# nicoRomeroCuruchet/DynamicProgramming

Hardware: AMD Instinct MI355X
Metric: state-action Bellman backups/sec (higher is better)
Workload: dtype f32; 1 GPU; double_pendulum_swingup 4D grid bins=80/dim (40960000 states) x 11 actions, gamma=0.999; step = 10 eval sweeps + 1 improve sweep = 860160000 backups; terminal states are counted in `value` (0 of 40960000: value_nonterminal leaves them out); states=40960000, nonterminal_states=40960000, actions=11, parallelism=state-range shards x1

## Files before the change

dynamicprogramming_amd/_native.py:

```python
from __future__ import annotations

import ctypes
import enum
import os
from pathlib import Path

import numpy as np

_PKG = Path(__file__).resolve().parent
LIB_PATH = _PKG / "libpi_mi355.so"
KERNEL_CACHE = Path(os.environ.get("PI_MI355_KERNEL_CACHE", str(_PKG / "_kcache")))

_f32p = ctypes.POINTER(ctypes.c_float)
_i32p = ctypes.POINTER(ctypes.c_int32)
_vp = ctypes.c_void_p

SIGNATURES = {
    "pi_abi_version": (ctypes.c_int, []),
    "pi_last_error": (ctypes.c_char_p, []),
    "pi_create": (_vp, [ctypes.c_int, ctypes.c_int, _i32p, _f32p, _f32p,
                        ctypes.POINTER(_f32p), _f32p, ctypes.c_int]),
    "pi_destroy": (None, [_vp]),
    "pi_compile": (ctypes.c_int, [_vp, ctypes.c_char_p, ctypes.c_char_p, ctypes.c_char_p,
                                  ctypes.c_size_t]),
    "pi_kernel_source": (ctypes.c_size_t, [_vp, ctypes.c_char_p, ctypes.c_char_p, ctypes.c_size_t]),
    "pi_eval_sweep": (ctypes.c_int, [_vp, _vp, _vp, _vp, _vp, ctypes.c_int64, ctypes.c_int64,
                                     ctypes.c_float, _vp, _vp]),
    "pi_eval_sweeps": (ctypes.c_int, [_vp, _vp, _vp, _vp, _vp, ctypes.c_int64, ctypes.c_int64,
                                      ctypes.c_float, ctypes.c_int, _vp, _vp]),
    "pi_policy_evaluation": (ctypes.c_int, [_vp, _vp, _vp, _vp, ctypes.c_float, ctypes.c_double, ctypes.c_int,
                                            ctypes.c_int, _vp, _vp, _vp, _vp]),
    "pi_policy_iteration": (ctypes.c_int, [_vp, _vp, _vp, _vp, ctypes.c_float, ctypes.c_double, ctypes.c_int,
                                           ctypes.c_int, ctypes.c_int, _vp, _vp, _vp]),
    "pi_improve_sweep": (ctypes.c_int, [_vp, _vp, _vp, _vp, ctypes.c_int64, ctypes.c_int64,
                                        ctypes.c_float, _vp, _vp]),
    "pi_value_sweep": (ctypes.c_int, [_vp, _vp, _vp, _vp, _vp, ctypes.c_int64, ctypes.c_int64,
                                      ctypes.c_float, _vp, _vp, _vp]),
    "pi_reach_planes": (ctypes.c_int, [_vp, _vp, ctypes.c_int64, ctypes.c_int64, ctypes.c_int, _vp, _vp]),
    "pi_reach_depth_max": (ctypes.c_int, [_vp]),
    "pi_reach_units": (ctypes.c_int, [_vp, _vp, ctypes.c_int64, ctypes.c_int64, ctypes.c_int, _vp, _vp]),
    "pi_comm_unique_id": (ctypes.c_int, [_vp]),
    "pi_comm_init": (ctypes.c_int, [_vp, ctypes.c_int, ctypes.c_int, _vp]),
    "pi_comm_init_local": (ctypes.c_int, [_vp, ctypes.c_int, ctypes.c_int, ctypes.c_char_p]),
    "pi_p2p_describe": (ctypes.c_int, [_vp, ctypes.c_int, ctypes.c_int, _vp, _vp, ctypes.c_int, _vp]),
    "pi_comm_init_p2p": (ctypes.c_int, [_vp, ctypes.c_int, ctypes.c_int, _vp, ctypes.c_char_p]),
    "pi_p2p_compile_check": (ctypes.c_int, [ctypes.c_char_p]),
    "pi_comm_destroy": (ctypes.c_int, [_vp]),
    "pi_comm_info": (ctypes.c_int, [_vp, ctypes.c_int]),
    "pi_allgather_V": (ctypes.c_int, [_vp, _vp, ctypes.c_int64, _vp]),
    "pi_allgather_policy": (ctypes.c_int, [_vp, _vp, ctypes.c_int64, _vp]),
# ... 16 lines not shown
    "pi_infer_destroy": (None, [_vp]),
    "pi_infer_set_policy": (ctypes.c_int, [_vp, _i32p, ctypes.c_int64, _f32p, ctypes.c_int]),
    "pi_infer_query": (ctypes.c_int, [_vp, _vp, ctypes.c_int64, _vp, _vp, _vp, _vp]),
    "pi_plan_schedule": (ctypes.c_int, [_vp, ctypes.c_int, ctypes.c_int64, ctypes.c_int64, ctypes.c_int64, ctypes.c_int,
                                        ctypes.POINTER(ctypes.c_uint64)]),
    "pi_set_option": (ctypes.c_int, [_vp, ctypes.c_int, ctypes.c_int64]),
    "pi_info": (ctypes.c_int64, [_vp, ctypes.c_int]),
    "pi_debug_report": (ctypes.c_int, [_vp, ctypes.POINTER(ctypes.c_uint32)]),
    "pi_prepare_mask": (ctypes.c_int, [_vp, _vp, _vp]),
    "pi_prepare_mask_range": (ctypes.c_int, [_vp, _vp, ctypes.c_int64, ctypes.c_int64, _vp]),
    "pi_live_list": (ctypes.c_int64, [_vp, _vp, ctypes.c_int64, _vp]),
    "pi_eval_begin": (ctypes.c_int, [_vp, _vp, _vp, _vp]),
    "pi_eval_end": (ctypes.c_int, [_vp]),
}

ABI_VERSION = 10
_lib = None
_load_error: Exception | None = None


class Info(enum.IntEnum):
    N_STATES = 0
    N_ACTIONS = 1
    DIMS = 2
    EVAL_CPW = 3
    EVAL_VGPRS = 4
    IMPROVE_VGPRS = 5
    COMPUTE_UNITS = 6
    CACHE_HIT = 7
    IMPROVE_CPW = 8
    CACHED_GRAPHS = 9
# ... 2 lines not shown
    IMPROVE_BLOCK = 12
    RESIDENT_STATES_PER_THREAD = 13
    RESIDENT_ENABLED = 14
    DEBUG_CHECKS = 15
    LIVE_STATES = 16
    EVAL_LIST_ENTRIES = 17
    MEMORY_ORDER = 18
    FLOW_WORKGROUPS = 19
    RECIPROCAL_DIV = 20
    XCD_ENABLED = 30
    XCD_EVALUATIONS = 31
    XCD_FALLBACKS = 32
    WHOLE_RUNS = 33
    WHOLE_RUN_AVAILABLE = 34
    STRIP_STATES = 35


class Option(enum.IntEnum):
    EVAL_CPW = 0
    IMPROVE_CPW = 1
    GRAPHS = 2
    RESIDENT = 3
    MEMORY_ORDER = 4
    BUILD_PUSH = 5
    KEEP_LIVE_LIST = 6
    STRIP_STATES = 7
    XCD_RUN_FAILED = 8


class XcdFailure(enum.IntEnum):
# ... 219 lines not shown
                          d_residual_log, stream=0):
        _check(lib().pi_policy_evaluation(self._h, V, policy, term, gamma, float(theta), int(max_sweeps),
                                          int(check_interval), d_sweeps, d_delta or None, d_residual_log,
                                          stream or None), "pi_policy_evaluation")

    def policy_iteration(self, V, policy, term, gamma, theta, max_eval_sweeps, check_interval, max_pi_iter, d_result,
                         d_iter_log, stream=0):
        _check(lib().pi_policy_iteration(self._h, V, policy, term, gamma, float(theta), int(max_eval_sweeps),
                                         int(check_interval), int(max_pi_iter), d_result, d_iter_log, stream or None),
               "pi_policy_iteration")

    def improve_sweep(self, V, policy, term, s_begin, s_end, gamma, d_changed=0, stream=0):
        _check(lib().pi_improve_sweep(self._h, V, policy, term, s_begin, s_end, gamma,
                                      d_changed or None, stream or None), "pi_improve_sweep")

    def value_sweep(self, V, Vnew, policy, term, s_begin, s_end, gamma, d_delta=0, d_changed=0, stream=0):
        _check(lib().pi_value_sweep(self._h, V, Vnew, policy, term, s_begin, s_end, gamma,
                                    d_delta or None, d_changed or None, stream or None), "pi_value_sweep")

    def reach_planes(self, term, s_begin, s_end, d_bitmap, stream=0, dim=0):
        _check(lib().pi_reach_planes(self._h, term, s_begin, s_end, int(dim), d_bitmap, stream or None),
               "pi_reach_planes")

    def reach_depth_max(self) -> int:
        return int(lib().pi_reach_depth_max(self._h))

    def reach_units(self, term, s_begin, s_end, depth, d_bitmap, stream=0):
        _check(lib().pi_reach_units(self._h, term, s_begin, s_end, int(depth), d_bitmap, stream or None),
               "pi_reach_units")

# ... 162 lines not shown
```

dynamicprogramming_amd/csrc/pi_api.cpp:

```cpp

#include "pi_internal.h"

#include <hip/hiprtc.h>

#include <algorithm>
#include <cmath>
#include <cstdio>
#include <cstdlib>
#include <cstring>
#include <fstream>
#include <map>
#include <mutex>
#include <sstream>
#include <sys/stat.h>
#include <unistd.h>

#ifndef PI_CSRC_DIR
#error "build with -DPI_CSRC_DIR=\"...\" and -DPI_INCLUDE_DIR=\"...\""
#endif
asm(".section .rodata\n"
    ".global pi_embedded_kernels\n"
    "pi_embedded_kernels:\n"
    ".incbin \"" PI_CSRC_DIR "/pi_sweep_kernels.hip\"\n"
    ".byte 0\n"
// ... 259 lines not shown
            }
        }
    }
    return Grid2{launch_blocks(block, count, cpw), 1u};
}

}

namespace {

using pi::Sched;
using pi::plan_launch;

unsigned int* delta_slots(pi_handle* h) { return h->d_slots; }
unsigned int* changed_slots(pi_handle* h) { return h->d_slots + kSlots; }

}

namespace pi {

int check_ready(const pi_handle* h) {
    if (!h) return fail("null handle");
    if (h->device < 0) return fail("host-only handle (device = -1) cannot launch kernels");
    if (!h->module) return fail("pi_compile has not been called on this handle");
    return 0;
}

int check_range(const pi_handle* h, int64_t s_begin, int64_t s_end) {
    if (s_begin < 0 || s_end < s_begin || s_end > h->n_states)
        return fail("state range [" + std::to_string(s_begin) + ", " + std::to_string(s_end) +
// ... 48 lines not shown
    for (int64_t w = a >> 6; w <= (b - 1) >> 6 && a < b; ++w) {
        uint64_t word = h->live_bits[(size_t)(w - word0)];
        while (word) {
            const int bit = __builtin_ctzll(word);
            word &= word - 1;
            const int64_t s = (w << 6) + bit;
            if (s >= a && s < b) out.push_back((int32_t)s);
        }
    }
}

int64_t live_list_total(const pi_handle* h, int64_t entries) {
    const int64_t range = h->live_hi - h->live_lo;
    if (range <= 0 || entries <= 0) return 0;
    return (int64_t)((double)entries * ((double)h->n_states / (double)range));
}

void drop_eval_list(pi_handle* h) {
    h->eval_count = -1;
    h->eval_policy = nullptr;
    h->eval_holds.clear();
}

int launch_eval_live(pi_handle* h, const float* V, float* Vnew, const int32_t* policy, int64_t first, int64_t count,
                     float gamma, bool want_delta, hipStream_t st, const int32_t* list, int64_t list_total) {
    if (count <= 0) return 0;
    const int32_t* live = (list ? list : h->d_live) + first;
    if (!list) list_total = live_list_total(h, h->live_count);
    long long cnt = count;
    const float* tab = h->d_tab;
// ... 125 lines not shown
    h->xcd = h->flow && xcd_wanted;
    h->xcd_ring = env_int("PI_MI355_XCD_RING", 64, 4, 1024);
    h->xcd_states = (int)(((n + 31) / 32 + 31) / 32 * 32);
    if (device >= 0) {
        pi::DeviceGuard guard(device);
        hipDeviceProp_t prop;
        hipError_t e = hipGetDeviceProperties(&prop, device);
        if (e == hipSuccess && std::string(prop.gcnArchName).rfind(kArch, 0) != 0) {
            fail(std::string("pi_create: device is ") + prop.gcnArchName +
                 ", this library is built for gfx950 only");
            return nullptr;
        }
        if (e == hipSuccess) e = hipMalloc((void**)&h->d_tab, h->tab.size() * sizeof(float));
        if (e == hipSuccess)
            e = hipMemcpy(h->d_tab, h->tab.data(), h->tab.size() * sizeof(float), hipMemcpyHostToDevice);
        if (e == hipSuccess) e = hipMalloc((void**)&h->d_slots, 2 * kSlots * sizeof(unsigned int));
        if (e == hipSuccess) e = hipMemset(h->d_slots, 0, 2 * kSlots * sizeof(unsigned int));
        if (e != hipSuccess) {
            fail(std::string("pi_create: ") + hipGetErrorString(e));
            if (h->d_tab) (void)hipFree(h->d_tab);
            if (h->d_slots) (void)hipFree(h->d_slots);
            return nullptr;
        }
        h->num_cu = prop.multiProcessorCount;
    } else {
        h->num_cu = 256;
    }
    return h.release();
}

void pi_destroy(pi_handle* h) {
    if (!h) return;
// ... 144 lines not shown
        (void)hipGetLastError();
        return fail("could not build the evaluation-sweep graph");
    }
    return 0;
}

}

extern "C" {

int pi_compile(pi_handle* h, const char* dynamics_src, const char* cache_dir, char* log,
               size_t log_len) {
    pi::fail("");
    if (log && log_len) log[0] = 0;
    if (!h || !dynamics_src) return fail("null argument");
    std::vector<char> image;
    if (pi::compile_image(build_source(h, dynamics_src), cache_dir, log, log_len, image, &h->cache_hit)) return 1;
    h->compiled = true;
    resolve_strip(h);
    h->dynamics_src = dynamics_src;
    h->has_cache_dir = cache_dir != nullptr;
    h->cache_dir = cache_dir ? cache_dir : "";
    return load_module(h, image);
}

int pi_eval_sweep(pi_handle* h, const float* V, float* Vnew, const int32_t* policy,
                  const uint8_t* term, int64_t s_begin, int64_t s_end, float gamma,
                  float* d_delta, void* stream) {
    if (check_ready(h) || check_range(h, s_begin, s_end)) return 1;
    if (!V || !Vnew || !policy) return fail("null device pointer");
    if (V == Vnew) return fail("V and Vnew must be different buffers (Jacobi sweep)");
    pi::DeviceGuard guard(h->device);
    hipStream_t st = (hipStream_t)stream;
    if (s_end == s_begin) {
        if (d_delta) PI_HIP(hipMemsetAsync(d_delta, 0, sizeof(float), st));
        return 0;
    }
    if (pi::launch_eval(h, V, Vnew, policy, term, s_begin, s_end, gamma, d_delta != nullptr, st)) return 1;
    return pi::finalize(h, d_delta, nullptr, st);
}

int pi_eval_sweeps(pi_handle* h, float* Va, float* Vb, const int32_t* policy,
                   const uint8_t* term, int64_t s_begin, int64_t s_end, float gamma,
                   int n_sweeps, float* d_delta, void* stream) {
    if (check_ready(h) || check_range(h, s_begin, s_end)) return 1;
    if (n_sweeps < 0) return fail("n_sweeps < 0");
    if (!Va || !Vb || !policy) return fail("null device pointer");
    if (Va == Vb) return fail("Va and Vb must be different buffers (Jacobi sweep)");
    if (n_sweeps == 0) return 0;
    pi::DeviceGuard guard(h->device);
    hipStream_t st = (hipStream_t)stream;
    if (s_end == s_begin) {
        if (d_delta) PI_HIP(hipMemsetAsync(d_delta, 0, sizeof(float), st));
        return 0;
    }
    if (h->f_resident && h->use_resident && n_sweeps >= 2 && s_begin == 0 && s_end == h->n_states) {
        const float* tab = h->d_tab;
        double theta = 0.0;
        int interval = 1;
        int* sweeps_out = nullptr;
// ... 31 lines not shown
            }
        }
        if (hit) {
            hit->stamp = ++h->graph_clock;
            PI_HIP(hipGraphLaunch(hit->exec, st));
            return 0;
        }
    }
    const bool live = pi::live_usable(h, term, s_begin, s_end);
    int64_t first = 0, count = 0;
    if (live) pi::live_span(h, s_begin, s_end, &first, &count);
    const bool shorter = live && h->eval_count >= 0 && policy == h->eval_policy && s_begin == 0 && s_end == h->n_states;
    auto holds = [&](const float* buf) {
        return std::find(h->eval_holds.begin(), h->eval_holds.end(), buf) != h->eval_holds.end();
    };
    for (int i = 0; i < n_sweeps; ++i) {
        const float* src = (i & 1) ? Vb : Va;
        float* dst = (i & 1) ? Va : Vb;
        const bool want = i == n_sweeps - 1 && d_delta != nullptr;
        int rc;
        if (i >= 1 && shorter && holds(src) && holds(dst)) {
            rc = pi::launch_eval_live(h, src, dst, policy, 0, h->eval_count, gamma, want, st, h->d_eval_list,
                                      pi::live_list_total(h, h->eval_count));
        } else {
            rc = i >= 1 && live ? pi::launch_eval_live(h, src, dst, policy, first, count, gamma, want, st)
                                : pi::launch_eval(h, src, dst, policy, term, s_begin, s_end, gamma, want, st, i >= 1);
            if (shorter && !holds(dst)) h->eval_holds.push_back(dst);
        }
        if (rc) return 1;
    }
    return pi::finalize(h, d_delta, nullptr, st);
// ... 51 lines not shown
                     "%u, last %u %u %u %u\n", w[8], w[9], w[10], w[11], w[16], w[17], w[18], w[19]);
    return 0;
}
}

int pi_policy_evaluation(pi_handle* h, float* V, const int32_t* policy, const uint8_t* term, float gamma,
                         double theta, int max_sweeps, int check_interval, int32_t* d_sweeps, float* d_delta,
                         float* d_residual_log, void* stream) {
    if (check_ready(h)) return 1;
    const bool lds = h->f_resident && h->use_resident;
    if (!lds && !h->f_flow)
        return fail("pi_policy_evaluation: this grid has no one-launch evaluation kernel "
                    "(PI_INFO_RESIDENT_STATES_PER_THREAD: LDS-resident, PI_INFO_FLOW_WORKGROUPS: dataflow)");
    if (!V || !policy || !d_sweeps || !d_residual_log) return fail("null device pointer");
    if (max_sweeps < 1 || check_interval < 1) return fail("max_sweeps and check_interval must be positive");
    pi::DeviceGuard guard(h->device);
    const float* tab = h->d_tab;
    if (h->f_xcd && !h->xcd_off) {
        hipStream_t st = (hipStream_t)stream;
        if (launch_xcd(h, V, const_cast<int32_t*>(policy), term, gamma, theta, max_sweeps, check_interval, 0, d_sweeps, d_delta,
                       d_residual_log, nullptr, st))
            return 1;
        int32_t done = 0;
        PI_HIP(hipMemcpyAsync(&done, d_sweeps, sizeof done, hipMemcpyDeviceToHost, st));
        PI_HIP(hipStreamSynchronize(st));
        ++h->xcd_used;
        if (xcd_trace(h, done)) return 1;
        if (done >= 0) return 0;
        if (++h->xcd_failed >= 2) h->xcd_off = true;
    }
// ... 34 lines not shown
    PI_HIP(hipModuleLaunchKernel(h->f_resident, 1, 1, 1, h->resident_block, 1, 1, 0, (hipStream_t)stream, args, nullptr));
    return 0;
}

int pi_policy_iteration(pi_handle* h, float* V, int32_t* policy, const uint8_t* term, float gamma, double theta,
                        int max_eval_sweeps, int check_interval, int max_pi_iter, int32_t* d_result, uint32_t* d_iter_log,
                        void* stream) {
    if (check_ready(h)) return 1;
    const bool xcd = h->f_xcd && !h->xcd_off;
    const bool resident = !xcd && h->f_run_resident && h->use_resident;
    if (!resident && !xcd) return fail("pi_policy_iteration: this grid has no one-launch run (PI_INFO_WHOLE_RUN_AVAILABLE)");
    if (!V || !policy || !d_result || !d_iter_log) return fail("null device pointer");
    if (max_eval_sweeps < 1 || check_interval < 1 || max_pi_iter < 1) return fail("limits and check_interval must be positive");
    pi::DeviceGuard guard(h->device);
    pi::drop_eval_list(h);
    if (resident) {
        const float* tab = h->d_tab;
        void* args[] = {&V, &policy, &term, &tab, &gamma, &max_eval_sweeps, &theta, &check_interval, &max_pi_iter, &d_result,
                        &d_iter_log};
        PI_HIP(hipModuleLaunchKernel(h->f_run_resident, 1, 1, 1, h->resident_block, 1, 1, 0, (hipStream_t)stream, args, nullptr));
        ++h->whole_runs;
        return 0;
    }
    if (launch_xcd(h, V, policy, term, gamma, theta, max_eval_sweeps, check_interval, max_pi_iter, d_result, nullptr, nullptr,
                   d_iter_log, (hipStream_t)stream))
        return 1;
    ++h->whole_runs;
    if (std::getenv("PI_MI355_XCD_TRACE")) {
        int32_t done = 0;
        PI_HIP(hipMemcpyAsync(&done, d_result, sizeof done, hipMemcpyDeviceToHost, (hipStream_t)stream));
// ... 3 lines not shown
    return 0;
}

int pi_improve_sweep(pi_handle* h, const float* V, int32_t* policy, const uint8_t* term,
                     int64_t s_begin, int64_t s_end, float gamma, uint32_t* d_changed,
                     void* stream) {
    if (check_ready(h) || check_range(h, s_begin, s_end)) return 1;
    if (!V || !policy) return fail("null device pointer");
    pi::DeviceGuard guard(h->device);
    hipStream_t st = (hipStream_t)stream;
    if (s_end == s_begin) {
        if (d_changed) PI_HIP(hipMemsetAsync(d_changed, 0, sizeof(uint32_t), st));
        return 0;
    }
    pi::drop_eval_list(h);
    long long b = s_begin, e = s_end;
    const float* tab = h->d_tab;
    unsigned int* cslots = d_changed ? changed_slots(h) : nullptr;
    Sched sc;
    if (pi::live_usable(h, term, s_begin, s_end)) {
        int64_t first = 0, cnt = 0;
        pi::live_span(h, s_begin, s_end, &first, &cnt);
        if (cnt > 0) {
            const int32_t* live = h->d_live + first;
            long long count = cnt;
            const pi::Grid2 blocks = plan_launch(h, h->block_improve, first, cnt, pi::live_list_total(h, h->live_count),
                                                h->cpw_improve, &sc);
            void* largs[] = {&V, &policy, &live, &tab, &count, &gamma, &cslots, &sc};
            PI_HIP(hipModuleLaunchKernel(h->f_improve_live, blocks.x, blocks.y, 1, h->block_improve, 1, 1, 0, st, largs, nullptr));
        }
        return pi::finalize(h, nullptr, d_changed, st);
    }
    const pi::Grid2 blocks = plan_launch(h, h->block_improve, s_begin, s_end - s_begin, h->n_states, h->cpw_improve, &sc);
    void* args[] = {&V, &policy, &term, &tab, &b, &e, &gamma, &cslots, &sc};
    PI_HIP(hipModuleLaunchKernel(h->f_improve, blocks.x, blocks.y, 1, h->block_improve, 1, 1, 0, st, args, nullptr));
    return pi::finalize(h, nullptr, d_changed, st);
}

int pi_value_sweep(pi_handle* h, const float* V, float* Vnew, int32_t* policy, const uint8_t* term,
                   int64_t s_begin, int64_t s_end, float gamma, float* d_delta, uint32_t* d_changed,
                   void* stream) {
    if (check_ready(h) || check_range(h, s_begin, s_end)) return 1;
    if (!V || !Vnew || !policy) return fail("null device pointer");
    if (V == Vnew) return fail("V and Vnew must be different buffers (Jacobi sweep)");
    pi::drop_eval_list(h);
    pi::DeviceGuard guard(h->device);
    hipStream_t st = (hipStream_t)stream;
    if (s_end == s_begin) {
        if (d_delta) PI_HIP(hipMemsetAsync(d_delta, 0, sizeof(float), st));
        if (d_changed) PI_HIP(hipMemsetAsync(d_changed, 0, sizeof(uint32_t), st));
        return 0;
    }
    long long b = s_begin, e = s_end;
    const float* tab = h->d_tab;
    unsigned int* dbits = d_delta ? delta_slots(h) : nullptr;
    unsigned int* cslots = d_changed ? changed_slots(h) : nullptr;
    Sched sc;
    const pi::Grid2 blocks = plan_launch(h, h->block_improve, s_begin, s_end - s_begin, h->n_states, h->cpw_improve, &sc);
    void* args[] = {&V, &Vnew, &policy, &term, &tab, &b, &e, &gamma, &dbits, &cslots, &sc};
    PI_HIP(hipModuleLaunchKernel(h->f_value, blocks.x, blocks.y, 1, h->block_improve, 1, 1, 0, st, args, nullptr));
// ... 91 lines not shown

int pi_plan_schedule(pi_handle* h, int block, int64_t first, int64_t count, int64_t total, int chunks_per_workgroup,
                     uint64_t* out6) {
    if (!h || !out6) return fail("null argument");
    if (block < 64 || block > 1024 || (block & (block - 1)) || chunks_per_workgroup < 1 || chunks_per_workgroup > 64 ||
        first < 0 || count < 1 || total < 0)
        return fail("pi_plan_schedule: bad launch shape");
    Sched sc;
    const pi::Grid2 grid = plan_launch(h, block, first, count, total, chunks_per_workgroup, &sc);
    out6[0] = grid.x; out6[1] = grid.y; out6[2] = sc.period; out6[3] = sc.phase; out6[4] = (uint64_t)sc.cpw; out6[5] = 0;
    return 0;
}

int pi_set_option(pi_handle* h, int what, int64_t value) {
    if (!h) return fail("null handle");
    switch (what) {
        case PI_OPTION_EVAL_CPW:
            if (value < 1 || value > 64) return fail("chunks per workgroup must be in [1, 64]");
            h->cpw_eval = (int)value;
            drop_graphs(h);
            return 0;
        case PI_OPTION_IMPROVE_CPW:
            if (value < 1 || value > 64) return fail("chunks per workgroup must be in [1, 64]");
            h->cpw_improve = (int)value;
            return 0;
        case PI_OPTION_GRAPHS:
            h->use_graphs = value != 0;
            return 0;
        case PI_OPTION_RESIDENT:
            h->use_resident = value != 0;
// ... 49 lines not shown
            return 0;
        default:
            return fail("unknown option");
    }
}

int pi_prepare_mask(pi_handle* h, const uint8_t* d_term, void* stream) {
    if (pi::check_ready(h)) return 1;
    return pi_prepare_mask_range(h, d_term, 0, h->n_states, stream);
}

int pi_prepare_mask_range(pi_handle* h, const uint8_t* d_term, int64_t s_begin, int64_t s_end, void* stream) {
    if (pi::check_ready(h)) return 1;
    if (s_begin < 0 || s_end < s_begin || s_end > h->n_states) return fail("bad state range");
    pi::DeviceGuard guard(h->device);
    if (h->d_live) { (void)hipFree(h->d_live); h->d_live = nullptr; }
    if (h->d_eval_list) { (void)hipFree(h->d_eval_list); h->d_eval_list = nullptr; }
    if (h->d_eval_cursor) { (void)hipFree(h->d_eval_cursor); h->d_eval_cursor = nullptr; }
    pi::drop_eval_list(h);
    h->live_term = nullptr;
    h->live_count = 0;
    h->live_bits.clear();
    h->live_bits.shrink_to_fit();
    h->live_before.clear();
    h->live_before.shrink_to_fit();
    h->live_lo = h->live_hi = 0;
    if (!d_term || s_end == s_begin) return 0;
    const int64_t n = s_end - s_begin;
    if (h->n_states < env_int("PI_MI355_LIVE_MIN", 1 << 20, 1, 1 << 30) || !env_int("PI_MI355_LIVE", 1, 0, 1)) return 0;
    hipStream_t st = (hipStream_t)stream;
// ... 59 lines not shown
    if (pi::check_ready(h)) return -1;
    if (h->live_count <= 0 || !h->d_live) return 0;
    if (!d_out) return h->live_count;
    if (capacity < h->live_count) { fail("pi_live_list: capacity below the list's length"); return -1; }
    pi::DeviceGuard guard(h->device);
    if (hipMemcpyAsync(d_out, h->d_live, (size_t)h->live_count * sizeof(int32_t), hipMemcpyDeviceToDevice,
                       (hipStream_t)stream) != hipSuccess) { fail("pi_live_list: copy failed"); return -1; }
    return h->live_count;
}

int pi_eval_begin(pi_handle* h, const int32_t* policy, const uint8_t* term, void* stream) {
    if (pi::check_ready(h)) return 1;
    if (!policy) return fail("null device pointer");
    pi::drop_eval_list(h);
    if (!pi::live_usable(h, term, 0, h->n_states) || !env_int("PI_MI355_EVAL_LIST", 1, 0, 1)) return 0;
    pi::DeviceGuard guard(h->device);
    hipStream_t st = (hipStream_t)stream;
    const long long nblocks = (h->live_count + pi::kProbeBlock - 1) / pi::kProbeBlock;
    if (!h->d_eval_list) PI_HIP(hipMalloc((void**)&h->d_eval_list, (size_t)h->live_count * sizeof(int32_t)));
    if (!h->d_eval_cursor) PI_HIP(hipMalloc((void**)&h->d_eval_cursor, (size_t)(nblocks + 1) * sizeof(unsigned long long)));
    const int32_t* live = h->d_live;
    long long count = h->live_count;
    const float* tab = h->d_tab;
    int32_t* out = h->d_eval_list;
    unsigned long long* slots = h->d_eval_cursor;
    for (int pass = 0; pass < 2; ++pass) {
        void* args[] = {&live, &count, &policy, &tab, &slots, &out, &pass};
        PI_HIP(hipModuleLaunchKernel(h->f_policy_list, (unsigned)nblocks, 1, 1, pi::kProbeBlock, 1, 1, 0, st, args, nullptr));
        if (pass == 0) {
            long long nb = nblocks;
// ... 53 lines not shown
        case PI_INFO_LIVE_STATES: return h->live_count;
        case PI_INFO_EVAL_LIST_ENTRIES: return h->eval_count < 0 ? 0 : h->eval_count;
        case PI_INFO_MEMORY_ORDER: {
            int64_t code = 0;
            for (int k = h->D - 1; k >= 0; --k) code = (code << 3) | h->user_of_mem[k];
            return code;
        }
        case PI_INFO_FLOW_WORKGROUPS:
            return h->f_flow ? (h->n_states + h->flow_block - 1) / h->flow_block : (h->flow && h->device < 0 ? 1 : 0);
        case PI_INFO_XCD_ENABLED: return h->f_xcd && !h->xcd_off ? 1 : 0;
        case PI_INFO_XCD_EVALUATIONS: return h->xcd_used;
        case PI_INFO_XCD_FALLBACKS: return h->xcd_failed;
        case PI_INFO_WHOLE_RUNS: return h->whole_runs;
        case PI_INFO_WHOLE_RUN_AVAILABLE: return (h->f_run_resident && h->use_resident) || (h->f_xcd && !h->xcd_off) ? 1 : 0;
        case PI_INFO_STRIP_STATES: return h->strip_states;
        default:
            if (what >= PI_INFO_RECIPROCAL_DIV && what < PI_INFO_RECIPROCAL_DIV + h->D)
                return h->fastdiv[what - PI_INFO_RECIPROCAL_DIV];
            return -1;
    }
}

}
```

dynamicprogramming_amd/csrc/pi_comm.cpp:

```cpp

#include "pi_internal.h"

#include <rccl/rccl.h>

#include <algorithm>
#include <array>
#include <chrono>
#include <condition_variable>
#include <cstdlib>
#include <cstring>
#include <deque>
#include <map>
#include <mutex>

using pi::fail;

namespace pi {

struct ShardPlan {
    int64_t per = 0, s_begin = 0, s_end = 0;
    bool halo = false;
    int depth = 1;
    struct Seg { int src, dst; int64_t a, b; };
    std::vector<Seg> segs;
// ... 278 lines not shown
    int allreduce_sum_u32(uint32_t* d, hipStream_t st) override {
        uint32_t v;
        PI_HIP(hipMemcpyAsync(&v, d, sizeof v, hipMemcpyDeviceToHost, st));
        PI_HIP(hipStreamSynchronize(st));
        double r;
        if (reduce_host((double)v, false, &r)) return 1;
        v = (uint32_t)r;
        PI_HIP(hipMemcpyAsync(d, &v, sizeof v, hipMemcpyHostToDevice, st));
        PI_HIP(hipStreamSynchronize(st));
        return 0;
    }
};

int need_comm(pi_handle* h) {
    if (pi::check_ready(h)) return 1;
    if (!h->comm) return fail("no communicator on this handle: call pi_comm_init first");
    return 0;
}
int need_plan(pi_handle* h) {
    if (need_comm(h)) return 1;
    if (!h->plan) return fail("no exchange plan on this handle: call pi_exchange_plan first");
    if (h->plan->broken)
        return fail("a sharded sweep failed on this handle and its exchange was abandoned; the communicator is not usable "
                    "any more (RCCL: aborted; in-process: its group gave up).  Recover on EVERY rank: pi_comm_destroy, a new "
                    "pi_comm_init (fresh id) / pi_comm_init_local (fresh group name), then pi_exchange_plan");
    return 0;
}

int post_exchange(pi_handle* h, float* full, hipStream_t st) {
    pi::Comm* c = h->comm;
// ... 629 lines not shown
```

dynamicprogramming_amd/csrc/pi_internal.h:

```cpp
#pragma once

#include "pi_mi355.h"

#include <hip/hip_runtime.h>

#include <cstdint>
#include <memory>
#include <string>
#include <vector>

namespace pi {

int fail(const std::string& msg);
const std::string& last_error();

#define PI_HIP(expr)                                                                      \
    do {                                                                                  \
        hipError_t e_ = (expr);                                                           \
        if (e_ != hipSuccess)                                                             \
            return ::pi::fail(std::string(#expr) + ": " + hipGetErrorString(e_));         \
    } while (0)

constexpr int kProbeBlock = 256;
constexpr int kXcds = 8;
// ... 30 lines not shown
    virtual int push_wait(hipStream_t) { return 1; }
    virtual int push_wait_deferred(hipStream_t st) { return push_wait(st); }
};
struct ShardPlan;
struct P2pPending;

struct GraphEntry {
    const void *Va = nullptr, *Vb = nullptr, *policy = nullptr, *term = nullptr, *d_delta = nullptr;
    int64_t s_begin = 0, s_end = 0;
    float gamma = 0.0f;
    int n_sweeps = 0;
    hipGraphExec_t exec = nullptr;
    uint64_t stamp = 0;
};

}

struct pi_handle {
    int device = -1;
    int D = 0;
    int n_actions = 0;
    int64_t n_states = 0;
    std::vector<int32_t> shape;
    std::vector<float> lo, span, rcp;
    std::vector<int> fastdiv;
    std::vector<int> mem_of_user, user_of_mem;
    bool compiled = false;
    std::vector<float> tab;
    float* d_tab = nullptr;
    unsigned int* d_slots = nullptr;
    hipModule_t module = nullptr;
    hipModule_t module_push = nullptr;
    hipFunction_t f_eval_push = nullptr, f_reach_pairs = nullptr;
    std::string dynamics_src, cache_dir;
    bool has_cache_dir = false;
    hipFunction_t f_eval = nullptr, f_eval_live = nullptr, f_policy_list = nullptr, f_scan_slots = nullptr, f_mask_list = nullptr, f_improve = nullptr, f_improve_live = nullptr, f_value = nullptr, f_finalize = nullptr,
                  f_reach_planes = nullptr, f_reach_units = nullptr, f_probe_step = nullptr, f_probe_interp = nullptr,
                  f_probe_coords = nullptr, f_resident = nullptr, f_run_resident = nullptr;
    int num_cu = 0;
    int block_eval = 256, block_improve = 256;
    int cpw_eval = 1, cpw_improve = 1;
    int64_t strip_states = 0;
    int64_t strip_mode = -1;
    int vgpr_eval = -1, vgpr_improve = -1;
    bool cache_hit = false;
// ... 48 lines not shown
                     float gamma, bool want_delta, hipStream_t st, const int32_t* list = nullptr, int64_t list_total = 0);
int64_t live_list_total(const pi_handle* h, int64_t entries);
struct Sched {
    int cpw;
    unsigned int period, phase;
};
struct Grid2 { unsigned x, y; };
Grid2 plan_launch(const pi_handle* h, int block, int64_t first, int64_t count, int64_t total, int cpw, Sched* sc);
int ensure_push_module(pi_handle* h);
int launch_eval_push(pi_handle* h, const float* V, float* Vnew, const int32_t* policy, const int32_t* list,
                     const uint8_t* dest, float* const* d_peers, int n_peers, int64_t count, float gamma, bool want_delta,
                     hipStream_t st);
bool pairs_possible(const pi_handle* h);
int reach_pairs(pi_handle* h, const uint8_t* term, int64_t s_begin, int64_t s_end, uint32_t* d_bitmap, hipStream_t st);
void drop_eval_list(pi_handle* h);
void release_comm(pi_handle* h);
void drop_p2p_pending(pi_handle* h);
double comm_timeout_seconds();
int compile_image(const std::string& src, const char* cache_dir, char* log, size_t log_len,
                  std::vector<char>& image, bool* cache_hit);

}
```

dynamicprogramming_amd/solver.py:

```python
from __future__ import annotations

import abc
import logging
import os
import time
from dataclasses import dataclass
from itertools import product
from pathlib import Path

import numpy as np

from . import _native
from ._native import Info, Option, XcdFailure

try:
    from loguru import logger
except ImportError:
    logger = logging.getLogger("dynamicprogramming_amd")
    if not hasattr(logger, "success"):
        logger.success = logger.info


def _gpu_available() -> bool:
    if not _native.available():
# ... 120 lines not shown
        bits = bitmap.cpu().numpy().view(np.uint32)
        return ((bits[np.arange(n_planes) >> 5] >> (np.arange(n_planes) & 31).astype(np.uint32)) & 1).astype(bool)

    def reach_units(self, term, s_begin, s_end, depth):
        n_units = int(np.prod(self.engine._shape[:depth]))
        bitmap = self.torch.zeros((n_units + 31) // 32, dtype=self.torch.int32, device=self.device)
        self.engine.reach_units(self._ptr(term), s_begin, s_end, depth, bitmap.data_ptr(), self._stream())
        bits = bitmap.cpu().numpy().view(np.uint32)
        return ((bits[np.arange(n_units) >> 5] >> (np.arange(n_units) & 31).astype(np.uint32)) & 1).astype(bool)

    def improve_sweep(self, V, policy, term, s_begin, s_end, gamma, d_changed):
        self.engine.improve_sweep(V.data_ptr(), policy.data_ptr(), self._ptr(term), s_begin, s_end,
                                  gamma, 0 if d_changed is None else d_changed.data_ptr(),
                                  self._stream())

    def value_sweep(self, V, Vnew, policy, term, s_begin, s_end, gamma, d_delta, d_changed):
        self.engine.value_sweep(V.data_ptr(), Vnew.data_ptr(), policy.data_ptr(), self._ptr(term),
                                s_begin, s_end, gamma, 0 if d_delta is None else d_delta.data_ptr(),
                                0 if d_changed is None else d_changed.data_ptr(), self._stream())

    def close(self):
        self.xcd_evaluations, self.xcd_fallbacks, self.whole_runs = (
            self.engine.info(k) for k in (Info.XCD_EVALUATIONS, Info.XCD_FALLBACKS, Info.WHOLE_RUNS))
        self.engine.close()


def _native_reason() -> str:
    try:
        _native.lib()
        return ""
    except _native.NativeError as exc:
        return str(exc)


class _CudaPolicyIterationBase(abc.ABC):

    _D: int = 0
    MEMORY_ORDER = None
# ... 142 lines not shown
            if D == 4:
                for slow in rest:
                    out.append(tuple([slow] + [k for k in rest if k != slow] + [lane]))
        seen, uniq = set(), []
        for o in out:
            if o not in seen:
                seen.add(o)
                uniq.append(o)
        return uniq

    def _tune_memory_order(self, sweeps: int = 3):
        import hashlib
        import json
        import os
        import torch
        D, n = self._D, self.n_states
        dev = torch.device("cuda", torch.cuda.current_device() if self._device_arg is None
                           else torch.device(self._device_arg).index or 0)
        src = self._dynamics_cuda_src()
        key = hashlib.sha256()
        for part in (_native.kernel_source_hash().encode(), src.encode(), np.asarray(self.action_space, np.float32).tobytes(),
                     *[b.tobytes() for b in self._bins]):
            key.update(part)
            key.update(b"|")
        cache = _native.KERNEL_CACHE / f"order_{key.hexdigest()[:24]}.json"
        if os.environ.get("PI_MI355_ORDER_CACHE", "1") != "0" and cache.exists():
            try:
                rec = json.loads(cache.read_text())
                order = tuple(int(v) for v in rec["order"])
                if sorted(order) == list(range(D)):
# ... 154 lines not shown
            if self._comm.halo_elems >= 0:
                logger.info(f"halo exchange: rank {self._rank} receives "
                            f"{self._comm.halo_elems * 4 / 2**20:.1f} MiB per sweep instead of "
                            f"{(self._n_pad - self._shard_len) * 4 / 2**20:.1f} MiB")
        logger.success("Kernels compiled. Device memory allocated.")

    def _mask_arg(self):
        if hasattr(self, "_term_arg"):
            return self._term_arg
        return self.d_terminal_mask

    def _seed_values(self, mask: np.ndarray, value: float) -> None:
        import torch
        m = torch.from_numpy(np.ascontiguousarray(self._to_memory(np.ascontiguousarray(mask, dtype=bool)))).to(
            self.d_value_function.device)
        self.d_value_function[: self.n_states][m] = float(value)
        self.d_new_value_function[: self.n_states][m] = float(value)

    def _init_sharding(self) -> None:
        from . import transport as T
        comm = self._transport_arg
        if comm is False:
            comm = None
        elif comm is None:
            try:
                import torch.distributed as dist
                active = dist.is_available() and dist.is_initialized()
            except Exception:
                active = False
            if active and dist.get_world_size(self._process_group) > 1:
                comm = T.from_environment(self._process_group)
        self._comm = comm
        self._world, self._rank = (comm.world, comm.rank) if comm is not None else (1, 0)
        self._shard_len, self._s_begin, self._s_end = T.shard_bounds(self.n_states, self._rank, self._world)
        self._n_pad = self._shard_len * self._world
        if comm is not None:
            comm.attach(self)
            logger.info(f"rank {self._rank}/{self._world}: states [{self._s_begin:,}, {self._s_end:,})")

    def _evaluation_sweeps(self, n: int, gamma: float) -> None:
        if self._comm is not None:
            self._comm.evaluation_sweeps(self, n, gamma)
            return
        self._backend.eval_sweeps(self.d_value_function, self.d_new_value_function, self.d_policy,
                                  self._mask_arg(), self._s_begin, self._s_end, gamma, n,
                                  self._d_delta)
        if n & 1:
            self.d_value_function, self.d_new_value_function = (
                self.d_new_value_function, self.d_value_function)

    def _improvement_sweep(self, gamma: float) -> None:
        if self._comm is not None:
            self._comm.improvement_sweep(self, gamma)
            return
        self._backend.improve_sweep(self.d_value_function, self.d_policy, self._mask_arg(),
                                    self._s_begin, self._s_end, gamma, self._d_changed)

    def policy_evaluation(self) -> float:
        cfg = self.config
        gamma = float(np.float32(cfg.gamma))
        delta = float("inf")
        t0 = time.perf_counter()
        if self._comm is None and getattr(self._backend, "resident", False) and cfg.max_eval_iter >= 1:
            delta = self._policy_evaluation_resident(gamma, t0)
            if delta is not None:
                return delta
            delta = float("inf")
        i = 0
# ... 105 lines not shown
        self.stats["stable"] = stable
        self._d_delta.fill_(log[-1][1])
        if stable:
            logger.success(f"Policy Iteration converged at iteration {rounds}.")
        else:
            logger.warning(f"Policy Iteration hit max_pi_iter={cfg.max_pi_iter}.")
        self.stats["eval_seconds"] += time.perf_counter() - t0
        return True

    def value_iteration(self, max_iter: int | None = None) -> float:
        cfg = self.config
        gamma = float(np.float32(cfg.gamma))
        limit = cfg.max_eval_iter if max_iter is None else int(max_iter)
        delta = float("inf")
        sweeps = 0
        for i in range(limit):
            check = i % SYNC_INTERVAL == 0 or i == limit - 1
            self._backend.value_sweep(self.d_value_function, self.d_new_value_function, self.d_policy,
                                      self._mask_arg(), self._s_begin, self._s_end, gamma,
                                      self._d_delta if check else None, None)
            if self._comm is not None:
                self._comm.exchange(self, self.d_new_value_function)
            self.d_value_function, self.d_new_value_function = (
                self.d_new_value_function, self.d_value_function)
            sweeps += 1
            if check:
                if self._comm is not None:
                    self._comm.all_reduce_max(self, self._d_delta)
                delta = float(self._d_delta.item())
                if delta < cfg.theta:
# ... 19 lines not shown
                     grid_shape=self.grid_shape,
                     action_space=self.action_space,
                     eval_sweeps=np.int64(self.stats["eval_sweeps"]),
                     improve_sweeps=np.int64(self.stats["improve_sweeps"]),
                     pi_iterations=np.int64(self.stats["pi_iterations"]),
                     sweeps_per_iter=np.asarray(self.stats["sweeps_per_iter"], dtype=np.int64))
            os.replace(tmp, filepath)

    def load_checkpoint(self, filepath) -> None:
        import torch
        data = np.load(Path(filepath).with_suffix(".npz"))
        if not (np.array_equal(data["grid_shape"], self.grid_shape)
                and np.array_equal(data["action_space"], self.action_space)):
            raise ValueError("checkpoint was written for a different grid or action set")
        n, dev = self.n_states, self.d_value_function.device
        self.d_value_function[:n].copy_(torch.from_numpy(np.ascontiguousarray(self._to_memory(data["value_function"]))).to(dev))
        self.d_new_value_function.copy_(self.d_value_function)
        self.d_policy[:n].copy_(torch.from_numpy(np.ascontiguousarray(self._to_memory(data["policy"]))).to(dev))
        for key in ("eval_sweeps", "improve_sweeps", "pi_iterations"):
            self.stats[key] = int(data[key])
        if "sweeps_per_iter" in data:
            self.stats["sweeps_per_iter"] = [int(x) for x in data["sweeps_per_iter"]]

    def _pull_tensors_from_gpu(self) -> None:
        logger.info("Pulling results from device memory...")
        if self._comm is not None:
            self._comm.all_gather(self, self.d_policy)
            self._comm.all_gather(self, self.d_value_function)
        n = self.n_states
        self.value_function = np.ascontiguousarray(self._to_user(self.d_value_function[:n].cpu().numpy()))
# ... 47 lines not shown
```

include/pi_mi355.h:

```cpp
#ifndef PI_MI355_H_
#define PI_MI355_H_

#include <stddef.h>
#include <stdint.h>

#ifdef __cplusplus
extern "C" {
#endif

typedef struct pi_handle pi_handle;

#define PI_MI355_ABI_VERSION 10
int pi_abi_version(void);

const char* pi_last_error(void);

pi_handle* pi_create(int device, int D, const int32_t* grid_shape, const float* lo,
                     const float* hi, const float* const* bins, const float* actions,
                     int n_actions);
void pi_destroy(pi_handle* h);

int pi_compile(pi_handle* h, const char* dynamics_src, const char* cache_dir, char* log,
               size_t log_len);

size_t pi_kernel_source(pi_handle* h, const char* dynamics_src, char* buf, size_t buf_len);

int pi_eval_sweep(pi_handle* h, const float* V, float* Vnew, const int32_t* policy,
// ... 10 lines not shown

int pi_eval_begin(pi_handle* h, const int32_t* policy, const uint8_t* term, void* stream);
int pi_eval_end(pi_handle* h);

int pi_policy_evaluation(pi_handle* h, float* V, const int32_t* policy, const uint8_t* term, float gamma,
                         double theta, int max_sweeps, int check_interval, int32_t* d_sweeps, float* d_delta,
                         float* d_residual_log, void* stream);

int pi_policy_iteration(pi_handle* h, float* V, int32_t* policy, const uint8_t* term, float gamma, double theta,
                        int max_eval_sweeps, int check_interval, int max_pi_iter, int32_t* d_result, uint32_t* d_iter_log,
                        void* stream);

int pi_improve_sweep(pi_handle* h, const float* V, int32_t* policy, const uint8_t* term,
                     int64_t s_begin, int64_t s_end, float gamma, uint32_t* d_changed,
                     void* stream);

int pi_value_sweep(pi_handle* h, const float* V, float* Vnew, int32_t* policy, const uint8_t* term,
                   int64_t s_begin, int64_t s_end, float gamma, float* d_delta, uint32_t* d_changed,
                   void* stream);

int pi_reach_planes(pi_handle* h, const uint8_t* term, int64_t s_begin, int64_t s_end, int dim,
                    uint32_t* d_bitmap, void* stream);

int pi_reach_depth_max(pi_handle* h);
int pi_reach_units(pi_handle* h, const uint8_t* term, int64_t s_begin, int64_t s_end, int depth,
                   uint32_t* d_bitmap, void* stream);


int pi_comm_unique_id(void* id128);
int pi_comm_init(pi_handle* h, int rank, int world, const void* id128);
// ... 103 lines not shown
    PI_INFO_EVAL_BLOCK = 11,
    PI_INFO_IMPROVE_BLOCK = 12,
    PI_INFO_RESIDENT_STATES_PER_THREAD = 13,
    PI_INFO_RESIDENT_ENABLED = 14,
    PI_INFO_DEBUG_CHECKS = 15,
    PI_INFO_LIVE_STATES = 16,
    PI_INFO_EVAL_LIST_ENTRIES = 17,
    PI_INFO_MEMORY_ORDER = 18,
    PI_INFO_FLOW_WORKGROUPS = 19,
    PI_INFO_RECIPROCAL_DIV = 20,
    PI_INFO_XCD_ENABLED = 30,
    PI_INFO_XCD_EVALUATIONS = 31,
    PI_INFO_XCD_FALLBACKS = 32,
    PI_INFO_WHOLE_RUNS = 33,
    PI_INFO_WHOLE_RUN_AVAILABLE = 34,
    PI_INFO_STRIP_STATES = 35
};
int64_t pi_info(pi_handle* h, int what);

int pi_debug_report(pi_handle* h, uint32_t* out4);

#ifdef __cplusplus
}
#endif
#endif
```

Before: 146.5 billion backups/s.

## Fuse the first evaluation sweep into the improvement sweep via a carried Vnext

The improvement step now runs the value kernel, which writes the greedy max backup into Vnext while updating the policy. That max equals one evaluation backup under the new policy. The next pi_eval_sweeps call therefore skips its first sweep when the carry matches: same buffers, range, gamma and stream, and no intervening mutation. This removes one full grid sweep per policy-iteration step. In exchange it adds carry bookkeeping and invalidation across every API entry point and Python-side tensor version checks, and a small risk of stale results if some mutation path is missed.

New measurement: 153.0 billion backups/s (median of 6 runs). +4.4%, better.

```diff
diff --git a/dynamicprogramming_amd/_native.py b/dynamicprogramming_amd/_native.py
--- a/dynamicprogramming_amd/_native.py
+++ b/dynamicprogramming_amd/_native.py
@@ -34,6 +34,9 @@
                                            ctypes.c_int, ctypes.c_int, _vp, _vp, _vp]),
     "pi_improve_sweep": (ctypes.c_int, [_vp, _vp, _vp, _vp, ctypes.c_int64, ctypes.c_int64,
                                         ctypes.c_float, _vp, _vp]),
+    "pi_improve_sweep_carry": (ctypes.c_int, [_vp, _vp, _vp, _vp, _vp, ctypes.c_int64, ctypes.c_int64,
+                                              ctypes.c_float, _vp, _vp]),
+    "pi_carry_invalidate": (ctypes.c_int, [_vp]),
     "pi_value_sweep": (ctypes.c_int, [_vp, _vp, _vp, _vp, _vp, ctypes.c_int64, ctypes.c_int64,
                                       ctypes.c_float, _vp, _vp, _vp]),
     "pi_reach_planes": (ctypes.c_int, [_vp, _vp, ctypes.c_int64, ctypes.c_int64, ctypes.c_int, _vp, _vp]),
@@ -80,7 +83,7 @@
     "pi_eval_end": (ctypes.c_int, [_vp]),
 }
 
-ABI_VERSION = 10
+ABI_VERSION = 11
 _lib = None
 _load_error: Exception | None = None
 
@@ -113,6 +116,9 @@
     WHOLE_RUNS = 33
     WHOLE_RUN_AVAILABLE = 34
     STRIP_STATES = 35
+    CARRIES_ARMED = 40
+    CARRIES_USED = 41
+    CARRIES_DROPPED = 42
 
 
 class Option(enum.IntEnum):
@@ -362,6 +368,13 @@
         _check(lib().pi_improve_sweep(self._h, V, policy, term, s_begin, s_end, gamma,
                                       d_changed or None, stream or None), "pi_improve_sweep")
 
+    def improve_sweep_carry(self, V, Vnext, policy, term, s_begin, s_end, gamma, d_changed=0, stream=0):
+        _check(lib().pi_improve_sweep_carry(self._h, V, Vnext, policy, term, s_begin, s_end, gamma,
+                                            d_changed or None, stream or None), "pi_improve_sweep_carry")
+
+    def carry_invalidate(self) -> None:
+        _check(lib().pi_carry_invalidate(self._h), "pi_carry_invalidate")
+
     def value_sweep(self, V, Vnew, policy, term, s_begin, s_end, gamma, d_delta=0, d_changed=0, stream=0):
         _check(lib().pi_value_sweep(self._h, V, Vnew, policy, term, s_begin, s_end, gamma,
                                     d_delta or None, d_changed or None, stream or None), "pi_value_sweep")
diff --git a/dynamicprogramming_amd/csrc/pi_api.cpp b/dynamicprogramming_amd/csrc/pi_api.cpp
--- a/dynamicprogramming_amd/csrc/pi_api.cpp
+++ b/dynamicprogramming_amd/csrc/pi_api.cpp
@@ -297,6 +297,7 @@
 
 unsigned int* delta_slots(pi_handle* h) { return h->d_slots; }
 unsigned int* changed_slots(pi_handle* h) { return h->d_slots + kSlots; }
+float* carried_delta(pi_handle* h) { return reinterpret_cast<float*>(h->d_slots + 2 * kSlots); }
 
 }
 
@@ -375,6 +376,11 @@
     const int64_t range = h->live_hi - h->live_lo;
     if (range <= 0 || entries <= 0) return 0;
     return (int64_t)((double)entries * ((double)h->n_states / (double)range));
+}
+
+void drop_carry(pi_handle* h) {
+    if (h->carry.armed) ++h->carries_dropped;
+    h->carry.armed = false;
 }
 
 void drop_eval_list(pi_handle* h) {
@@ -530,8 +536,8 @@
         if (e == hipSuccess) e = hipMalloc((void**)&h->d_tab, h->tab.size() * sizeof(float));
         if (e == hipSuccess)
             e = hipMemcpy(h->d_tab, h->tab.data(), h->tab.size() * sizeof(float), hipMemcpyHostToDevice);
-        if (e == hipSuccess) e = hipMalloc((void**)&h->d_slots, 2 * kSlots * sizeof(unsigned int));
-        if (e == hipSuccess) e = hipMemset(h->d_slots, 0, 2 * kSlots * sizeof(unsigned int));
+        if (e == hipSuccess) e = hipMalloc((void**)&h->d_slots, (2 * kSlots + 1) * sizeof(unsigned int));
+        if (e == hipSuccess) e = hipMemset(h->d_slots, 0, (2 * kSlots + 1) * sizeof(unsigned int));
         if (e != hipSuccess) {
             fail(std::string("pi_create: ") + hipGetErrorString(e));
             if (h->d_tab) (void)hipFree(h->d_tab);
@@ -706,6 +712,7 @@
     pi::fail("");
     if (log && log_len) log[0] = 0;
     if (!h || !dynamics_src) return fail("null argument");
+    pi::drop_carry(h);
     std::vector<char> image;
     if (pi::compile_image(build_source(h, dynamics_src), cache_dir, log, log_len, image, &h->cache_hit)) return 1;
     h->compiled = true;
@@ -722,6 +729,7 @@
     if (check_ready(h) || check_range(h, s_begin, s_end)) return 1;
     if (!V || !Vnew || !policy) return fail("null device pointer");
     if (V == Vnew) return fail("V and Vnew must be different buffers (Jacobi sweep)");
+    pi::drop_carry(h);
     pi::DeviceGuard guard(h->device);
     hipStream_t st = (hipStream_t)stream;
     if (s_end == s_begin) {
@@ -735,7 +743,22 @@
 int pi_eval_sweeps(pi_handle* h, float* Va, float* Vb, const int32_t* policy,
                    const uint8_t* term, int64_t s_begin, int64_t s_end, float gamma,
                    int n_sweeps, float* d_delta, void* stream) {
-    if (check_ready(h) || check_range(h, s_begin, s_end)) return 1;
+    if (check_ready(h)) return 1;
+    const pi::Carry was = h->carry;
+    h->carry.armed = false;
+    const float gamma_f = gamma;
+    uint32_t gamma_bits;
+    std::memcpy(&gamma_bits, &gamma_f, sizeof gamma_bits);
+    bool carried = was.armed && !h->comm && n_sweeps >= 1 && was.V == Va && was.Vnext == Vb && was.policy == policy &&
+                   was.term == term && was.s_begin == s_begin && was.s_end == s_end && was.gamma_bits == gamma_bits &&
+                   was.stream == (hipStream_t)stream;
+    if (was.armed && !carried) ++h->carries_dropped;
+    if (check_range(h, s_begin, s_end)) { if (carried) ++h->carries_dropped; return 1; }
+    struct CarryOutcome {
+        pi_handle* h;
+        bool pending;
+        ~CarryOutcome() { if (pending) ++h->carries_dropped; }
+    } outcome{h, carried};
     if (n_sweeps < 0) return fail("n_sweeps < 0");
     if (!Va || !Vb || !policy) return fail("null device pointer");
     if (Va == Vb) return fail("Va and Vb must be different buffers (Jacobi sweep)");
@@ -797,7 +820,18 @@
     auto holds = [&](const float* buf) {
         return std::find(h->eval_holds.begin(), h->eval_holds.end(), buf) != h->eval_holds.end();
     };
-    for (int i = 0; i < n_sweeps; ++i) {
+    int first_sweep = 0;
+    if (carried) {
+        if (live) return fail("pi_eval_sweeps: a carry met a live-state list (internal error)");
+        outcome.pending = false;
+        ++h->carries_used;
+        first_sweep = 1;
+        if (n_sweeps == 1) {
+            if (d_delta) PI_HIP(hipMemcpyAsync(d_delta, carried_delta(h), sizeof(float), hipMemcpyDeviceToDevice, st));
+            return 0;
+        }
+    }
+    for (int i = first_sweep; i < n_sweeps; ++i) {
         const float* src = (i & 1) ? Vb : Va;
         float* dst = (i & 1) ? Va : Vb;
         const bool want = i == n_sweeps - 1 && d_delta != nullptr;
@@ -879,6 +913,7 @@
                     "(PI_INFO_RESIDENT_STATES_PER_THREAD: LDS-resident, PI_INFO_FLOW_WORKGROUPS: dataflow)");
     if (!V || !policy || !d_sweeps || !d_residual_log) return fail("null device pointer");
     if (max_sweeps < 1 || check_interval < 1) return fail("max_sweeps and check_interval must be positive");
+    pi::drop_carry(h);
     pi::DeviceGuard guard(h->device);
     const float* tab = h->d_tab;
     if (h->f_xcd && !h->xcd_off) {
@@ -943,6 +978,7 @@
     if (max_eval_sweeps < 1 || check_interval < 1 || max_pi_iter < 1) return fail("limits and check_interval must be positive");
     pi::DeviceGuard guard(h->device);
     pi::drop_eval_list(h);
+    pi::drop_carry(h);
     if (resident) {
         const float* tab = h->d_tab;
         void* args[] = {&V, &policy, &term, &tab, &gamma, &max_eval_sweeps, &theta, &check_interval, &max_pi_iter, &d_result,
@@ -976,6 +1012,7 @@
         return 0;
     }
     pi::drop_eval_list(h);
+    pi::drop_carry(h);
     long long b = s_begin, e = s_end;
     const float* tab = h->d_tab;
     unsigned int* cslots = d_changed ? changed_slots(h) : nullptr;
@@ -999,6 +1036,43 @@
     return pi::finalize(h, nullptr, d_changed, st);
 }
 
+int pi_improve_sweep_carry(pi_handle* h, const float* V, float* Vnext, int32_t* policy, const uint8_t* term,
+                           int64_t s_begin, int64_t s_end, float gamma, uint32_t* d_changed, void* stream) {
+    if (check_ready(h) || check_range(h, s_begin, s_end)) return 1;
+    if (!V || !Vnext || !policy) return fail("null device pointer");
+    if (V == Vnext) return fail("V and Vnext must be different buffers (Jacobi sweep)");
+    if (h->comm || s_end == s_begin || pi::live_usable(h, term, s_begin, s_end))
+        return pi_improve_sweep(h, V, policy, term, s_begin, s_end, gamma, d_changed, stream);
+    pi::drop_eval_list(h);
+    pi::drop_carry(h);
+    pi::DeviceGuard guard(h->device);
+    hipStream_t st = (hipStream_t)stream;
+    long long b = s_begin, e = s_end;
+    const float* tab = h->d_tab;
+    unsigned int* dbits = delta_slots(h);
+    unsigned int* cslots = d_changed ? changed_slots(h) : nullptr;
+    Sched sc;
+    const pi::Grid2 blocks = plan_launch(h, h->block_improve, s_begin, s_end - s_begin, h->n_states, h->cpw_improve, &sc);
+    void* args[] = {&V, &Vnext, &policy, &term, &tab, &b, &e, &gamma, &dbits, &cslots, &sc};
+    PI_HIP(hipModuleLaunchKernel(h->f_value, blocks.x, blocks.y, 1, h->block_improve, 1, 1, 0, st, args, nullptr));
+    if (pi::finalize(h, carried_delta(h), d_changed, st)) return 1;
+    pi::Carry& c = h->carry;
+    c.armed = true;
+    c.V = V; c.Vnext = Vnext; c.policy = policy; c.term = term;
+    c.s_begin = s_begin; c.s_end = s_end;
+    const float gamma_f = gamma;
+    std::memcpy(&c.gamma_bits, &gamma_f, sizeof c.gamma_bits);
+    c.stream = st;
+    ++h->carries_armed;
+    return 0;
+}
+
+int pi_carry_invalidate(pi_handle* h) {
+    if (!h) return fail("null handle");
+    pi::drop_carry(h);
+    return 0;
+}
+
 int pi_value_sweep(pi_handle* h, const float* V, float* Vnew, int32_t* policy, const uint8_t* term,
                    int64_t s_begin, int64_t s_end, float gamma, float* d_delta, uint32_t* d_changed,
                    void* stream) {
@@ -1006,6 +1080,7 @@
     if (!V || !Vnew || !policy) return fail("null device pointer");
     if (V == Vnew) return fail("V and Vnew must be different buffers (Jacobi sweep)");
     pi::drop_eval_list(h);
+    pi::drop_carry(h);
     pi::DeviceGuard guard(h->device);
     hipStream_t st = (hipStream_t)stream;
     if (s_end == s_begin) {
@@ -1127,6 +1202,7 @@
 
 int pi_set_option(pi_handle* h, int what, int64_t value) {
     if (!h) return fail("null handle");
+    pi::drop_carry(h);
     switch (what) {
         case PI_OPTION_EVAL_CPW:
             if (value < 1 || value > 64) return fail("chunks per workgroup must be in [1, 64]");
@@ -1206,6 +1282,7 @@
     if (pi::check_ready(h)) return 1;
     if (s_begin < 0 || s_end < s_begin || s_end > h->n_states) return fail("bad state range");
     pi::DeviceGuard guard(h->device);
+    pi::drop_carry(h);
     if (h->d_live) { (void)hipFree(h->d_live); h->d_live = nullptr; }
     if (h->d_eval_list) { (void)hipFree(h->d_eval_list); h->d_eval_list = nullptr; }
     if (h->d_eval_cursor) { (void)hipFree(h->d_eval_cursor); h->d_eval_cursor = nullptr; }
@@ -1295,6 +1372,7 @@
     if (!policy) return fail("null device pointer");
     pi::drop_eval_list(h);
     if (!pi::live_usable(h, term, 0, h->n_states) || !env_int("PI_MI355_EVAL_LIST", 1, 0, 1)) return 0;
+    pi::drop_carry(h);
     pi::DeviceGuard guard(h->device);
     hipStream_t st = (hipStream_t)stream;
     const long long nblocks = (h->live_count + pi::kProbeBlock - 1) / pi::kProbeBlock;
@@ -1378,6 +1456,9 @@
         case PI_INFO_WHOLE_RUNS: return h->whole_runs;
         case PI_INFO_WHOLE_RUN_AVAILABLE: return (h->f_run_resident && h->use_resident) || (h->f_xcd && !h->xcd_off) ? 1 : 0;
         case PI_INFO_STRIP_STATES: return h->strip_states;
+        case PI_INFO_CARRIES_ARMED: return h->carries_armed;
+        case PI_INFO_CARRIES_USED: return h->carries_used;
+        case PI_INFO_CARRIES_DROPPED: return h->carries_dropped;
         default:
             if (what >= PI_INFO_RECIPROCAL_DIV && what < PI_INFO_RECIPROCAL_DIV + h->D)
                 return h->fastdiv[what - PI_INFO_RECIPROCAL_DIV];
diff --git a/dynamicprogramming_amd/csrc/pi_comm.cpp b/dynamicprogramming_amd/csrc/pi_comm.cpp
--- a/dynamicprogramming_amd/csrc/pi_comm.cpp
+++ b/dynamicprogramming_amd/csrc/pi_comm.cpp
@@ -316,6 +316,7 @@
 
 int need_comm(pi_handle* h) {
     if (pi::check_ready(h)) return 1;
+    pi::drop_carry(h);
     if (!h->comm) return fail("no communicator on this handle: call pi_comm_init first");
     return 0;
 }
diff --git a/dynamicprogramming_amd/csrc/pi_internal.h b/dynamicprogramming_amd/csrc/pi_internal.h
--- a/dynamicprogramming_amd/csrc/pi_internal.h
+++ b/dynamicprogramming_amd/csrc/pi_internal.h
@@ -68,6 +68,17 @@
     uint64_t stamp = 0;
 };
 
+struct Carry {
+    bool armed = false;
+    const float* V = nullptr;
+    const float* Vnext = nullptr;
+    const int32_t* policy = nullptr;
+    const uint8_t* term = nullptr;
+    int64_t s_begin = 0, s_end = 0;
+    uint32_t gamma_bits = 0;
+    hipStream_t stream = nullptr;
+};
+
 }
 
 struct pi_handle {
@@ -83,6 +94,8 @@
     std::vector<float> tab;
     float* d_tab = nullptr;
     unsigned int* d_slots = nullptr;
+    pi::Carry carry;
+    int64_t carries_armed = 0, carries_used = 0, carries_dropped = 0;
     hipModule_t module = nullptr;
     hipModule_t module_push = nullptr;
     hipFunction_t f_eval_push = nullptr, f_reach_pairs = nullptr;
@@ -161,6 +174,7 @@
 bool pairs_possible(const pi_handle* h);
 int reach_pairs(pi_handle* h, const uint8_t* term, int64_t s_begin, int64_t s_end, uint32_t* d_bitmap, hipStream_t st);
 void drop_eval_list(pi_handle* h);
+void drop_carry(pi_handle* h);
 void release_comm(pi_handle* h);
 void drop_p2p_pending(pi_handle* h);
 double comm_timeout_seconds();
diff --git a/dynamicprogramming_amd/solver.py b/dynamicprogramming_amd/solver.py
--- a/dynamicprogramming_amd/solver.py
+++ b/dynamicprogramming_amd/solver.py
@@ -158,6 +158,13 @@
                                   gamma, 0 if d_changed is None else d_changed.data_ptr(),
                                   self._stream())
 
+    def improve_sweep_carry(self, V, Vnext, policy, term, s_begin, s_end, gamma, d_changed):
+        self.engine.improve_sweep_carry(V.data_ptr(), Vnext.data_ptr(), policy.data_ptr(), self._ptr(term), s_begin,
+                                        s_end, gamma, 0 if d_changed is None else d_changed.data_ptr(), self._stream())
+
+    def carry_invalidate(self) -> None:
+        self.engine.carry_invalidate()
+
     def value_sweep(self, V, Vnew, policy, term, s_begin, s_end, gamma, d_delta, d_changed):
         self.engine.value_sweep(V.data_ptr(), Vnew.data_ptr(), policy.data_ptr(), self._ptr(term),
                                 s_begin, s_end, gamma, 0 if d_delta is None else d_delta.data_ptr(),
@@ -166,6 +173,7 @@
     def close(self):
         self.xcd_evaluations, self.xcd_fallbacks, self.whole_runs = (
             self.engine.info(k) for k in (Info.XCD_EVALUATIONS, Info.XCD_FALLBACKS, Info.WHOLE_RUNS))
+        self.carries = tuple(self.engine.info(k) for k in (Info.CARRIES_ARMED, Info.CARRIES_USED, Info.CARRIES_DROPPED))
         self.engine.close()
 
 
@@ -338,6 +346,7 @@
         import json
         import os
         import torch
+        self.drop_carry()
         D, n = self._D, self.n_states
         dev = torch.device("cuda", torch.cuda.current_device() if self._device_arg is None
                            else torch.device(self._device_arg).index or 0)
@@ -522,6 +531,7 @@
         import torch
         m = torch.from_numpy(np.ascontiguousarray(self._to_memory(np.ascontiguousarray(mask, dtype=bool)))).to(
             self.d_value_function.device)
+        self.drop_carry()
         self.d_value_function[: self.n_states][m] = float(value)
         self.d_new_value_function[: self.n_states][m] = float(value)
 
@@ -546,10 +556,36 @@
             comm.attach(self)
             logger.info(f"rank {self._rank}/{self._world}: states [{self._s_begin:,}, {self._s_end:,})")
 
+    _CARRY_TENSORS = ("d_value_function", "d_new_value_function", "d_policy")
+
+    def _carry_enabled(self) -> bool:
+        return (os.environ.get("PI_MI355_CARRY", "1") != "0" and self._comm is None
+                and hasattr(self._backend, "improve_sweep_carry"))
+
+    def _carry_state(self):
+        tensors = [getattr(self, name, None) for name in self._CARRY_TENSORS] + [self._mask_arg()]
+        return [(t, None if t is None else t._version) for t in tensors]
+
+    def drop_carry(self) -> None:
+        if getattr(self, "_carry_snapshot", None) is not None:
+            self._carry_snapshot = None
+            self._backend.carry_invalidate()
+
+    def _check_carry(self) -> None:
+        snap = getattr(self, "_carry_snapshot", None)
+        if snap is None:
+            return
+        now = self._carry_state()
+        if any(a is not b or va != vb for (a, va), (b, vb) in zip(snap, now)):
+            self.drop_carry()
+        else:
+            self._carry_snapshot = None
+
     def _evaluation_sweeps(self, n: int, gamma: float) -> None:
         if self._comm is not None:
             self._comm.evaluation_sweeps(self, n, gamma)
             return
+        self._check_carry()
         self._backend.eval_sweeps(self.d_value_function, self.d_new_value_function, self.d_policy,
                                   self._mask_arg(), self._s_begin, self._s_end, gamma, n,
                                   self._d_delta)
@@ -560,6 +596,12 @@
     def _improvement_sweep(self, gamma: float) -> None:
         if self._comm is not None:
             self._comm.improvement_sweep(self, gamma)
+            return
+        if self._carry_enabled():
+            self._carry_snapshot = None
+            self._backend.improve_sweep_carry(self.d_value_function, self.d_new_value_function, self.d_policy,
+                                              self._mask_arg(), self._s_begin, self._s_end, gamma, self._d_changed)
+            self._carry_snapshot = self._carry_state()
             return
         self._backend.improve_sweep(self.d_value_function, self.d_policy, self._mask_arg(),
                                     self._s_begin, self._s_end, gamma, self._d_changed)
@@ -695,6 +737,7 @@
         limit = cfg.max_eval_iter if max_iter is None else int(max_iter)
         delta = float("inf")
         sweeps = 0
+        self.drop_carry()
         for i in range(limit):
             check = i % SYNC_INTERVAL == 0 or i == limit - 1
             self._backend.value_sweep(self.d_value_function, self.d_new_value_function, self.d_policy,
@@ -744,6 +787,7 @@
                 and np.array_equal(data["action_space"], self.action_space)):
             raise ValueError("checkpoint was written for a different grid or action set")
         n, dev = self.n_states, self.d_value_function.device
+        self.drop_carry()
         self.d_value_function[:n].copy_(torch.from_numpy(np.ascontiguousarray(self._to_memory(data["value_function"]))).to(dev))
         self.d_new_value_function.copy_(self.d_value_function)
         self.d_policy[:n].copy_(torch.from_numpy(np.ascontiguousarray(self._to_memory(data["policy"]))).to(dev))
diff --git a/include/pi_mi355.h b/include/pi_mi355.h
--- a/include/pi_mi355.h
+++ b/include/pi_mi355.h
@@ -10,7 +10,7 @@
 
 typedef struct pi_handle pi_handle;
 
-#define PI_MI355_ABI_VERSION 10
+#define PI_MI355_ABI_VERSION 11
 int pi_abi_version(void);
 
 const char* pi_last_error(void);
@@ -51,6 +51,10 @@
 int pi_improve_sweep(pi_handle* h, const float* V, int32_t* policy, const uint8_t* term,
                      int64_t s_begin, int64_t s_end, float gamma, uint32_t* d_changed,
                      void* stream);
+
+int pi_improve_sweep_carry(pi_handle* h, const float* V, float* Vnext, int32_t* policy, const uint8_t* term,
+                           int64_t s_begin, int64_t s_end, float gamma, uint32_t* d_changed, void* stream);
+int pi_carry_invalidate(pi_handle* h);
 
 int pi_value_sweep(pi_handle* h, const float* V, float* Vnew, int32_t* policy, const uint8_t* term,
                    int64_t s_begin, int64_t s_end, float gamma, float* d_delta, uint32_t* d_changed,
@@ -184,7 +188,10 @@
     PI_INFO_XCD_FALLBACKS = 32,
     PI_INFO_WHOLE_RUNS = 33,
     PI_INFO_WHOLE_RUN_AVAILABLE = 34,
-    PI_INFO_STRIP_STATES = 35
+    PI_INFO_STRIP_STATES = 35,
+    PI_INFO_CARRIES_ARMED = 40,
+    PI_INFO_CARRIES_USED = 41,
+    PI_INFO_CARRIES_DROPPED = 42
 };
 int64_t pi_info(pi_handle* h, int what);
 
```
